# huangnengCSU/NanoSNP

Measured on AMD Instinct MI355X. Metric: candidate SNP sites/sec (pileup encode + model fwd), 30x windows, higher is better.
Workload: dtype f32; 1 GPU; BASELINE configs[1]: pileup encode + PileupModel fwd, 1M synthetic 30x windows (G2) resident in HBM, batch=4096; batch=4096, windows_resident_per_gpu=1048576, streams=32, precision=fp32, parallelism=site-sharded x1, rooted gather of calls, world_size_observed=1, gather=torch

## Files before the change

### nanosnp_amd/csrc/nsnp_api.hip

```cpp
#include "nsnp_common.hpp"

#include <new>

extern "C" int nsnp_version(void) { return 101; }

extern "C" const char* nsnp_strerror(int code)
{
    switch (code) {
    case NSNP_OK: return "ok";
    case NSNP_EINVAL: return "invalid argument";
    case NSNP_ENOMEM: return "out of memory";
    case NSNP_EHIP: return "HIP runtime error";
    case NSNP_ENOWEIGHTS: return "weights not loaded";
    case NSNP_EARCH: return "device is not gfx950";
    case NSNP_ESHAPE: return "unsupported model dimensions";
    case NSNP_ENOTSUP: return "optional component unavailable (RCCL not found)";
    case NSNP_ECOMM: return "RCCL call failed";
    default: return "unknown error";
    }
}

static hipError_t g_create_err = hipSuccess;

extern "C" int nsnp_last_hip_error(const nsnp_ctx* ctx, const char** text)
{
    const hipError_t e = ctx ? ctx->last_err : g_create_err;
    if (text) *text = hipGetErrorString(e);
    return (int)e;
}

extern "C" int nsnp_ctx_create(int device, nsnp_ctx** out)
{
    if (!out) return NSNP_EINVAL;
    *out = nullptr;
    nsnp_ctx* ctx = new (std::nothrow) nsnp_ctx();
    if (!ctx) return NSNP_ENOMEM;
    memset((void*)ctx, 0, sizeof(*ctx));
    ctx->device = device;
    ctx->last_err = hipSuccess;
    ctx->chunk_sites = 32768;
    ctx->hap_chunk = 16384;
    ctx->precision = 0;
    ctx->hap_precision = 0;
    ctx->cat_precision = 0;
    ctx->cat_conv_lds = 1;
    ctx->cat_conv_pix2 = 1;
    ctx->hap_b3x = 1;
    ctx->tok_fused = 0;
    ctx->proj1_tiles = 4;
    ctx->fused_l1 = 1;
    ctx->l0_rs = 2;
    ctx->l1_rs = 1;
    ctx->l1_stagger = 0;
    ctx->l1_weave = 1;
    ctx->head_rs = 1;
    ctx->rs_prio = 0;
    hipDeviceProp_t prop;
    hipError_t e = hipSetDevice(device);
    if (e == hipSuccess) e = hipGetDeviceProperties(&prop, device);
    if (e != hipSuccess) { g_create_err = e; delete ctx; return NSNP_EHIP; }
    if (strncmp(prop.gcnArchName, "gfx950", 6) != 0) { delete ctx; return NSNP_EARCH; }
    ctx->n_cu = prop.multiProcessorCount;
    *out = ctx;
    return NSNP_OK;
}

void nsnp_hap_free(nsnp_ctx* ctx);
int  nsnp_hap_reserve(nsnp_ctx* ctx);
void nsnp_cat_free(nsnp_ctx* ctx);
void nsnp_tok_free(nsnp_ctx* ctx);

constexpr size_t TIMER_MAX_PAIRS = 8192;

ScopedKernelTimer::ScopedKernelTimer(nsnp_ctx* c, int kernel, hipStream_t stream)
    : ctx(c), k(kernel), s(stream), stop_ev(nullptr), on(false)
{
    KernelTimer* t = c->timer;
    if (!t || !t->enabled || t->used[k] >= TIMER_MAX_PAIRS) return;
    if (t->used[k] == t->start[k].size()) {
        hipEvent_t a, b;
        if (hipEventCreate(&a) != hipSuccess) return;
        if (hipEventCreate(&b) != hipSuccess) { (void)hipEventDestroy(a); return; }
        t->start[k].push_back(a); t->stop[k].push_back(b);
    }
    const size_t i = t->used[k]++;
    (void)hipEventRecord(t->start[k][i], s);
    stop_ev = t->stop[k][i];
    on = true;
}
void ScopedKernelTimer::stop() { if (on) { (void)hipEventRecord(stop_ev, s); on = false; } }
ScopedKernelTimer::~ScopedKernelTimer() { stop(); }

extern "C" int nsnp_ctx_set_option(nsnp_ctx* ctx, const char* name, int64_t value)
{
    if (!ctx || !name) return NSNP_EINVAL;
    if (strcmp(name, "cat_precision") == 0) {
        if (value != 0 && value != 1 && value != 2) return NSNP_EINVAL;
        ctx->cat_precision = (int)value;
        return NSNP_OK;
    }
    if (strcmp(name, "tok_fused") == 0) {
        if (value != 0 && value != 1) return NSNP_EINVAL;
        ctx->tok_fused = (int)value;
        return NSNP_OK;
    }
    if (strcmp(name, "hap_b3x") == 0) {
        if (value != 0 && value != 1) return NSNP_EINVAL;
        ctx->hap_b3x = (int)value;
        return NSNP_OK;
    }
    if (strcmp(name, "cat_conv_pix2") == 0) {
        if (value != 0 && value != 1) return NSNP_EINVAL;
        ctx->cat_conv_pix2 = (int)value;
        return NSNP_OK;
    }
    if (strcmp(name, "cat_conv_lds") == 0) {
        if (value != 0 && value != 1) return NSNP_EINVAL;
        ctx->cat_conv_lds = (int)value;
        return NSNP_OK;
    }
    if (strcmp(name, "hap_precision") == 0) {
        if (value != 0 && value != 1 && value != 2) return NSNP_EINVAL;
        ctx->hap_precision = (int)value;
        return nsnp_hap_reserve(ctx);
    }
    if (strcmp(name, "hap_pass_sites") == 0) {
        if (value < 128 || value > 131072 || value % 128) return NSNP_EINVAL;
        const int64_t old = ctx->hap_chunk;
        ctx->hap_chunk = value;
        const int rc = nsnp_hap_reserve(ctx);
        if (rc) { ctx->hap_chunk = old; (void)nsnp_hap_reserve(ctx); }
        return rc;
    }
    if (strcmp(name, "pileup_precision") == 0) {
        if (value != 0 && value != 1 && value != 2) return NSNP_EINVAL;
        ctx->precision = (int)value;
        if (value == 2 && ctx->ws_h0 && ctx->ws_h0_floats < 192) return nsnp_ctx_reserve(ctx, ctx->chunk_sites);
        return NSNP_OK;
    }
    if (strcmp(name, "fused_l1") == 0) {
        if (value != 0 && value != 1) return NSNP_EINVAL;
        ctx->fused_l1 = (int)value;
        return NSNP_OK;
    }
    if (strcmp(name, "l0_register_stationary") == 0) {
        if (value != 0 && value != 1 && value != 2) return NSNP_EINVAL;
        ctx->l0_rs = (int)value;
        return NSNP_OK;
    }
    if (strcmp(name, "l1_register_stationary") == 0) {
        if (value != 0 && value != 1 && value != 2) return NSNP_EINVAL;
        ctx->l1_rs = (int)value;
        return NSNP_OK;
    }
    if (strcmp(name, "l0_input_weights_in_lds") == 0) {
        if (value != 0 && value != 1) return NSNP_EINVAL;
        ctx->l0_wx_lds = (int)value;
        return NSNP_OK;
    }
    if (strcmp(name, "static_priority") == 0) {
        if (value < 0 || value > 3) return NSNP_EINVAL;
        ctx->rs_prio = (int)value;
        return NSNP_OK;
    }
    if (strcmp(name, "head_split") == 0) {
        if (value != 0 && value != 1) return NSNP_EINVAL;
        ctx->head_rs = (int)value;
        return NSNP_OK;
    }
    if (strcmp(name, "l1_stagger") == 0) {
        if (value != 0 && value != 1) return NSNP_EINVAL;
        ctx->l1_stagger = (int)value;
        return NSNP_OK;
    }
    if (strcmp(name, "l1_weave") == 0) {
        if (value != 0 && value != 1) return NSNP_EINVAL;
        ctx->l1_weave = (int)value;
        return NSNP_OK;
    }
    if (strcmp(name, "l1_site_groups") == 0) {
        if (value != 0 && value != 1 && value != 2 && value != 4) return NSNP_EINVAL;
        ctx->l1_rs_groups = (int)value;
        return NSNP_OK;
    }
    if (strcmp(name, "l0_site_groups") == 0) {
        if (value != 0 && value != 1 && value != 2 && value != 4) return NSNP_EINVAL;
        ctx->l0_rs_groups = (int)value;
        return NSNP_OK;
    }
    if (strcmp(name, "fused_waves") == 0) {
        if (value != 0 && value != 4 && value != 8 && value != 12) return NSNP_EINVAL;
        ctx->fused_waves = (int)value;
        return NSNP_OK;
    }
    if (strcmp(name, "proj1_tiles") == 0) {
        if (value < 1 || value > 64) return NSNP_EINVAL;
        ctx->proj1_tiles = (int)value;
        return NSNP_OK;
    }
    if (strcmp(name, "recurrence_waves") == 0) {
        if (value != 0 && value != 1 && value != 2 && value != 4 && value != 8) return NSNP_EINVAL;
        ctx->force_wpb = (int)value;
        return NSNP_OK;
    }
    return NSNP_EINVAL;
}

extern "C" int nsnp_ctx_enable_timing(nsnp_ctx* ctx, int enable)
{
    if (!ctx) return NSNP_EINVAL;
    if (!ctx->timer) {
        ctx->timer = new (std::nothrow) KernelTimer();
        if (!ctx->timer) return NSNP_ENOMEM;
        for (int k = 0; k < NSNP_K_COUNT; ++k) ctx->timer->used[k] = 0;
    }
    ctx->timer->enabled = enable != 0;
    return NSNP_OK;
}

extern "C" int nsnp_ctx_read_timing(nsnp_ctx* ctx, int kernel, double* total_ms, int64_t* launches)
{
    if (!ctx || kernel < 0 || kernel >= NSNP_K_COUNT || !total_ms || !launches) return NSNP_EINVAL;
    *total_ms = 0.0; *launches = 0;
    KernelTimer* t = ctx->timer;
    if (!t) return NSNP_OK;
    for (size_t i = 0; i < t->used[kernel]; ++i) {
        NSNP_HIP(ctx, hipEventSynchronize(t->stop[kernel][i]));
        float ms = 0.f;
        NSNP_HIP(ctx, hipEventElapsedTime(&ms, t->start[kernel][i], t->stop[kernel][i]));
        *total_ms += ms; ++*launches;
    }
    t->used[kernel] = 0;
    return NSNP_OK;
}

static void free_ws(nsnp_ctx* ctx)
{
    if (ctx->ws_h0) (void)hipFree(ctx->ws_h0);
    if (ctx->ws_xp1) (void)hipFree(ctx->ws_xp1);
    if (ctx->ws_h1c) (void)hipFree(ctx->ws_h1c);
    ctx->ws_h0 = ctx->ws_xp1 = ctx->ws_h1c = nullptr;
    ctx->ws_h0_floats = 0;
}

extern "C" int nsnp_ctx_destroy(nsnp_ctx* ctx)
{
    if (!ctx) return NSNP_EINVAL;
    (void)hipSetDevice(ctx->device);
    (void)hipDeviceSynchronize();
    free_ws(ctx);
    if (ctx->pw.arena) (void)hipFree(ctx->pw.arena);
    if (ctx->pw16.arena) (void)hipFree(ctx->pw16.arena);
    if (ctx->pw16.l1f_bias) (void)hipFree(ctx->pw16.l1f_bias);
    if (ctx->pwb3.arena) (void)hipFree(ctx->pwb3.arena);
    if (ctx->sel_tmp) (void)hipFree(ctx->sel_tmp);
    if (ctx->fil_tmp) (void)hipFree(ctx->fil_tmp);
    if (ctx->rec_tmp) (void)hipFree(ctx->rec_tmp);
    if (ctx->lab_tmp) (void)hipFree(ctx->lab_tmp);
    if (ctx->evl_tmp) (void)hipFree(ctx->evl_tmp);
    if (ctx->pw.head6_w) (void)hipFree(ctx->pw.head6_w);
// ... 137 lines not shown
```

### nanosnp_amd/csrc/nsnp_common.hpp

```cpp
#pragma once

#include <hip/hip_runtime.h>
#include <stdint.h>
#include <stdlib.h>
#include <string.h>
#include <vector>

#include "nanosnp.h"

typedef float f32x4 __attribute__((ext_vector_type(4)));
typedef int   i32x4 __attribute__((ext_vector_type(4)));

#define NSNP_CDIV(a, b) (((a) + (b) - 1) / (b))

constexpr int PW = NSNP_PILEUP_WINDOW;
constexpr int PC = NSNP_PILEUP_CHANNELS;
constexpr int PH = 64;
constexpr int PG = 4 * PH;
constexpr int PCENTER = 16;
constexpr int PSTEPS1 = PCENTER + 1;


struct PileupWeightsDev {
    float* l0_whh[2];
    float* l0_wih[2];
    float* l0_wlast[2];
    void*  l0_wx[2];
    float* l1_wih[2];
    float* l1_bias[2];
    float* l1_bias_raw[2];
    float* l1_whh[2];
    float* proj_w;
    float* proj_b;
    float* dense_w;
    float* dense_b;
    float* head_w;
    float* head_b;
    float* arena;
    size_t arena_bytes;
    bool   loaded;
    float* head6_w;
    float* head6_b;
    bool   indel_loaded;
};

struct PileupWeightsF16 {
    void* l0_whh[2]; void* l0_wih_hi[2]; void* l0_wih_lo[2]; void* l1_wih[2]; void* l1_whh[2];
    void* l1f_hi[2]; void* l1f_lo[2]; float* l1f_bias;
    void* l0_wih_rs[2];
    void* l1_wih_rs[2]; void* l1_whh_rs[2];
    void* l0_whh_rs[2];
    void* proj_w; void* dense_w; void* head_w;
    void* arena; size_t arena_bytes; bool loaded;
};

struct PileupWeightsB3 {
    void* l0_whh[2]; void* l0_wih[2]; void* l1_wih[2]; void* l1_whh[2];
    void* proj_w; void* dense_w; void* head_w;
    float* proj_b; float* dense_b; float* head_b;
    void* arena; size_t arena_bytes; bool loaded;
};

struct HapWeightsDev;
struct CatWeightsDev;

enum { NSNP_K_L0 = 0, NSNP_K_PROJ1, NSNP_K_L1, NSNP_K_HEAD, NSNP_K_ENCODE, NSNP_K_HAPFEAT, NSNP_K_HAPLSTM, NSNP_K_CATCONV, NSNP_K_CAT,
       NSNP_K_COUNT };
struct KernelTimer {
    std::vector<hipEvent_t> start[NSNP_K_COUNT], stop[NSNP_K_COUNT];
    size_t used[NSNP_K_COUNT];
    bool enabled;
};

struct PostOut { uint8_t* gt_arg; uint8_t* zy_arg; float* gt_max; float* zy_max; };

struct nsnp_ctx {
    int device;
    int n_cu;
    hipError_t last_err;
    bool attr_set;
    bool attr_set_f16;
    bool attr_set_b3;
    int hap_b3x;
    int cat_conv_pix2;
    int cat_conv_lds;
    int cat_precision;
    int hap_precision;
    int precision;
    int fused_waves;
    int l0_rs;
    int l1_rs_groups;
    int l1_rs;
    int l0_rs_groups;
    int fused_l1;
    int proj1_tiles;
    int force_wpb;
    int l0_wx_lds;
    int rs_prio;
    int head_rs;
    int l1_stagger;
    int l1_weave;
    int64_t chunk_sites;
    float*  ws_h0;
    int     ws_h0_floats;
    float*  ws_xp1;
    float*  ws_h1c;
    PileupWeightsDev pw;
    PileupWeightsF16 pw16;
    PileupWeightsB3 pwb3;
    HapWeightsDev* hw;
    void*  hap_ws; size_t hap_ws_bytes; int64_t hap_ws_chunk;
    int64_t hap_chunk;
    CatWeightsDev* cw;
    void*  cat_ws; size_t cat_ws_bytes;
    int64_t* sel_tmp; size_t sel_tmp_bytes;
    int64_t* fil_tmp; size_t fil_tmp_bytes;
    void* rec_tmp; size_t rec_tmp_bytes;
    void* evl_tmp; size_t evl_tmp_bytes;
    void* lab_tmp; size_t lab_tmp_bytes;
    void* tok_ws; size_t tok_ws_bytes;
    void* ctg_ws; size_t ctg_ws_bytes;
    int tok_fused;
    bool af_cached; uint64_t af_bits, af_t; int af_k, af_mode; uint32_t af_table_words[128];
    bool af2_cached; uint64_t af2_bits, af2_t; int af2_k, af2_mode; uint32_t af2_table_words[128];
    KernelTimer* timer;
    void* comm; int comm_rank, comm_world;
    bool comm_borrowed;
};

struct ScopedKernelTimer {
    nsnp_ctx* ctx; int k; hipStream_t s; hipEvent_t stop_ev; bool on;
    ScopedKernelTimer(nsnp_ctx* c, int kernel, hipStream_t stream);
    void stop();
    ~ScopedKernelTimer();
};

#define NSNP_HIP(ctx, call)                                                        \
    do {                                                                           \
        hipError_t e_ = (call);                                                    \
        if (e_ != hipSuccess) { (ctx)->last_err = e_; return NSNP_EHIP; }          \
    } while (0)

typedef float (*nsnp_wfun)(const void* user, int row, int k);
void nsnp_pack_image(float* img, int n_tiles, int n_j4, nsnp_wfun f, const void* user);

int nsnp_ctx_need_xp1(nsnp_ctx* ctx);

int nsnp_pileup_forward_impl(nsnp_ctx* ctx, const int32_t* x, const int64_t* center_idx,
                             int64_t N, float* gt, float* zy, const PostOut* post, bool* post_written, hipStream_t s);
int nsnp_pileup_pack_weights(nsnp_ctx* ctx, const float* const* w);
int nsnp_pileup_pack_indel_heads(nsnp_ctx* ctx, const float* const* w);
int nsnp_pileup_eval_impl(nsnp_ctx* ctx, const int32_t* x, const int64_t* center_idx, const uint8_t* cls, int64_t N, float* site_loss,
                          uint8_t* pred, int64_t* counters, float* logits, hipStream_t s);
void nsnp_pileup_eval_heads_launch(nsnp_ctx* ctx, int64_t n, const uint8_t* cls, float* site_loss, uint8_t* pred, int64_t* counters,
                                   float* logits, hipStream_t s);
int nsnp_pileup_forward_f16x3(nsnp_ctx* ctx, const int32_t* x, const int64_t* center_idx,
                              int64_t N, float* gt, float* zy, hipStream_t s);
int nsnp_pileup_pack_weights_f16(nsnp_ctx* ctx, const float* const* w);
int nsnp_pileup_forward_bf16x3(nsnp_ctx* ctx, const int32_t* x, const int64_t* center_idx, int64_t N, float* gt, float* zy,
                               const PostOut* post, hipStream_t s);
int nsnp_pileup_pack_weights_bf16(nsnp_ctx* ctx, const float* const* w);
```

### nanosnp_amd/csrc/pileup_forward.hip

```cpp
#include "nsnp_common.hpp"
#include "nsnp_lstm_cell.hpp"
#include "nsnp_devclock.hpp"
#include "nsnp_bf16.hpp"
#include <type_traits>

namespace {

constexpr float LOG2E = 1.4426950408889634f;

__device__ __forceinline__ f32x4 mfma4(float a, float b, f32x4 c)
{
    return __builtin_amdgcn_mfma_f32_16x16x4f32(a, b, c, 0, 0, 0);
}
__device__ __forceinline__ float sigmoid_f(float x)
{
    return __builtin_amdgcn_rcpf(1.0f + __builtin_amdgcn_exp2f(-LOG2E * x));
}
__device__ __forceinline__ float tanh_f(float x)
{
    return __builtin_fmaf(-2.0f, __builtin_amdgcn_rcpf(1.0f + __builtin_amdgcn_exp2f((2.0f * LOG2E) * x)), 1.0f);
}

__device__ __forceinline__ float lstm_cell(float zi, float zf, float zg, float zo, float& c)
{
// ... 520 lines not shown
    for (int i = tid; i < 2 * 3 * RX_PLANE / 8; i += 256) reinterpret_cast<b8*>(&xx[0][0][0])[i] = b8{0, 0, 0, 0, 0, 0, 0, 0};
    if (tid < 8) xlvl[tid >> 2][tid & 3] = 0;
    __syncthreads();
    if (tid < 32) xx[tid >> 4][0][2 * 128 + (tid & 15) * 8 + 2] = (__bf16)1.0f;
    load_x(dir ? PW - 1 : 0);
    stage_x(0);
    if (PW > 1) load_x(dir ? PW - 2 : 1);
    __syncthreads();

    float c[4];
#pragma unroll
    for (int u = 0; u < 4; ++u) c[u] = 0.f;

    float* const h0wg = H0 + (base_site * PW * 2 + dir) * 64;
    const int frow = tid >> 4, fcid = tid & 15;
    unsigned foff = (unsigned)(frow * (PW * 128) + 4 * fcid) * 4u;
    const float* const fl = &hx[0][frow][16 * (fcid & 3) + 4 * (fcid >> 2)];
    const bool fon = frow < nrows;
    auto flush_h = [&](int buf, int t) {
        asm volatile("" : "+v"(foff));
        if (fon)
            *reinterpret_cast<f32x4*>(reinterpret_cast<char*>(h0wg + t * 128) + foff) =
                *reinterpret_cast<const f32x4*>(fl + buf * (16 * RS_XROW));
    };

    for (int s = 0; s < PW; ++s) {
        const int t = dir ? PW - 1 - s : s;
        const int cur = s & 1;
        if (s > 0) flush_h(cur ^ 1, dir ? t + 1 : t - 1);
        const __bf16* xr = &xx[cur][0][q * 128 + n * 8];
        const b8 xb0 = *reinterpret_cast<const b8*>(xr);
        const i32x4 lv = *reinterpret_cast<const i32x4*>(xlvl[cur]);
        const int lvl = __builtin_amdgcn_readfirstlane(max(max(lv[0], lv[1]), max(lv[2], lv[3])));
        f32x4 hn;
        auto step = [&](auto lvl_tag) __attribute__((always_inline)) {
            constexpr int LVL = decltype(lvl_tag)::value;
            const float* hr = &hx[cur ^ 1][n][4 * q];
            f32x4 hb0, hb1;
            if (s > 0) { hb0 = *reinterpret_cast<const f32x4*>(hr); hb1 = *reinterpret_cast<const f32x4*>(hr + 16); }
            f32x4 acc[4];
#pragma unroll
            for (int u = 0; u < 4; ++u) acc[u] = f32x4{0.f, 0.f, 0.f, 0.f};
#pragma unroll
            for (int p = LVL; p >= 0; --p) {
                const b8 b = p ? *reinterpret_cast<const b8*>(xr + p * RX_PLANE) : xb0;
#pragma unroll
                for (int wp = 2; wp >= 0; --wp)
#pragma unroll
                    for (int u = 0; u < 4; ++u) acc[u] = __builtin_amdgcn_mfma_f32_16x16x32_bf16(Wx[u][wp], b, acc[u], 0, 0, 0);
            }
            if (s > 0) {
#define RS_KBLOCK(J, HB)                                                                               \
                _Pragma("unroll") for (int e = 0; e < 4; ++e)                                          \
                    _Pragma("unroll") for (int u = 0; u < 4; ++u) acc[u] = mfma4(Whh[u][J][e], HB[e], acc[u]);
                __builtin_amdgcn_sched_barrier(0);
                RS_KBLOCK(0, hb0)
                __builtin_amdgcn_sched_barrier(0);
                hb0 = *reinterpret_cast<const f32x4*>(hr + 32);
                RS_KBLOCK(1, hb1)
                __builtin_amdgcn_sched_barrier(0);
                hb1 = *reinterpret_cast<const f32x4*>(hr + 48);
                RS_KBLOCK(2, hb0)
                __builtin_amdgcn_sched_barrier(0);
                RS_KBLOCK(3, hb1)
#undef RS_KBLOCK
            }
#pragma unroll
            for (int u = 0; u < 4; ++u) hn[u] = lstm_cell(acc[u][0], acc[u][1], acc[u][2], acc[u][3], c[u]);
        };
        if (__builtin_expect(lvl == 0, 1)) step(std::integral_constant<int, 0>{});
        else if (lvl == 1)                 step(std::integral_constant<int, 1>{});
        else                               step(std::integral_constant<int, 2>{});
        *reinterpret_cast<f32x4*>(&hx[cur][n][16 * wave + 4 * q]) = hn;
        if (s + 1 < PW) {
            stage_x(cur ^ 1);
            if (s + 2 < PW) load_x(dir ? t - 2 : t + 2);
        }
        lds_barrier();
    }
    flush_h((PW - 1) & 1, dir ? 0 : PW - 1);
    NSNP_DEVCLK_STOP(0)
}

constexpr int rs32_l1_lds_bytes(int nsg) { return (2 * 16 * nsg * RS_H0ROW + 2 * 16 * nsg * RS_XROW) * 4; }

template <int NSG, bool STAGGER>
__global__ __launch_bounds__(512, 2) void k_pileup_l1_rs32(
    const float* __restrict__ H0, int64_t N,
    const float* __restrict__ wih0, const float* __restrict__ wih1,
    const float* __restrict__ whh0, const float* __restrict__ whh1,
    const float* __restrict__ bias0, const float* __restrict__ bias1,
    float* __restrict__ H1c)
{
    extern __shared__ f32x4 lds[];
    constexpr int NS = 16 * NSG;
    float* const h0s = reinterpret_cast<float*>(lds);
    float* const h1x = h0s + 2 * NS * RS_H0ROW;
    const int dir = blockIdx.y;
    const int tid = threadIdx.x, lane = tid & 63, wave = tid >> 6;
    const int n = lane & 15, q = lane >> 4;
    const int64_t base_site = (int64_t)blockIdx.x * NS;

    f32x4 Wih[2][8], Whh[2][4], bias[2];
    {
        const f32x4* __restrict__ gih = reinterpret_cast<const f32x4*>(dir ? wih1 : wih0);
        const f32x4* __restrict__ ghh = reinterpret_cast<const f32x4*>(dir ? whh1 : whh0);
        const f32x4* __restrict__ gb = reinterpret_cast<const f32x4*>(dir ? bias1 : bias0);
#pragma unroll
        for (int u = 0; u < 2; ++u) {
#pragma unroll
            for (int j = 0; j < 8; ++j) Wih[u][j] = gih[((2 * wave + u) * 8 + j) * 64 + lane];
#pragma unroll
            for (int j = 0; j < 4; ++j) Whh[u][j] = ghh[((2 * wave + u) * 4 + j) * 64 + lane];
            bias[u] = gb[(2 * wave + u) * 64 + lane];
        }
    }

    const int cid = tid & 31;
    const int slot = (cid & 16) + 4 * (cid & 3) + ((cid >> 2) & 3);
    f32x4 sreg[NSG];
    auto load_h0 = [&](int t) {
#pragma unroll
        for (int k = 0; k < NSG; ++k) {
            const int64_t site = base_site + (tid >> 5) + 16 * k;
            const int64_t sc = site < N ? site : N - 1;
            sreg[k] = *reinterpret_cast<const f32x4*>(H0 + (sc * PW + t) * 128 + 4 * cid);
        }
    };
    auto store_h0 = [&](int buf) {
#pragma unroll
        for (int k = 0; k < NSG; ++k)
            *reinterpret_cast<f32x4*>(h0s + ((size_t)buf * NS + (tid >> 5) + 16 * k) * RS_H0ROW + 4 * slot) = sreg[k];
    };
    auto tpos = [&](int u) { return dir ? PW - 1 - u : u; };
    load_h0(tpos(0)); store_h0(0);
    load_h0(tpos(1)); store_h0(1);
    __syncthreads();
    load_h0(tpos(2));

    f32x4 acc[NSG][2];
    auto input_part = [&](int sg, int buf, f32x4& a0, f32x4& a1) {
        const float* r0 = h0s + ((size_t)buf * NS + 16 * sg + n) * RS_H0ROW + 4 * q;
        a0 = bias[0]; a1 = bias[1];
#pragma unroll
        for (int j = 0; j < 8; ++j) {
            const f32x4 b4 = *reinterpret_cast<const f32x4*>(r0 + 64 * (j >> 2) + 16 * (j & 3));
#pragma unroll
            for (int e = 0; e < 4; ++e) {
                a0 = mfma4(Wih[0][j][e], b4[e], a0);
                a1 = mfma4(Wih[1][j][e], b4[e], a1);
            }
        }
    };
    const bool late = STAGGER && wave >= 4;
#pragma unroll
    for (int sg = 0; sg < NSG; ++sg) input_part(sg, 0, acc[sg][0], acc[sg][1]);
    lds_barrier();

    float c[NSG][2];
#pragma unroll
    for (int sg = 0; sg < NSG; ++sg) c[sg][0] = c[sg][1] = 0.f;

    for (int s = 0; s < PSTEPS1; ++s) {
        const int cur = s & 1;
        const float* hrb = h1x + (size_t)(cur ^ 1) * NS * RS_XROW;
        float* hwb = h1x + (size_t)cur * NS * RS_XROW;
// ... 85 lines not shown
            const int64_t site = base_site + (tid >> 5) + 8 * k;
            const int64_t sc = site < N ? site : N - 1;
            sreg[k] = *reinterpret_cast<const f32x4*>(H0 + (sc * PW + t) * 128 + 4 * cid);
        }
    };
    auto store_h0 = [&](int buf) {
#pragma unroll
        for (int k = 0; k < 2 * NSG; ++k)
            *reinterpret_cast<f32x4*>(h0s + ((size_t)buf * NS + (tid >> 5) + 8 * k) * RS_H0ROW + 4 * slot) = sreg[k];
    };
    load_h0(dir ? PW - 1 : 0);
    store_h0(0);
    if (PSTEPS1 > 1) load_h0(dir ? PW - 2 : 1);
    __syncthreads();

    float c[NSG][4];
#pragma unroll
    for (int sg = 0; sg < NSG; ++sg)
#pragma unroll
        for (int u = 0; u < 4; ++u) c[sg][u] = 0.f;

    for (int s = 0; s < PSTEPS1; ++s) {
        const int t = dir ? PW - 1 - s : s;
        const int cur = s & 1;
        const float* h0b = h0s + (size_t)cur * NS * RS_H0ROW;
        const float* hrb = h1x + (size_t)(cur ^ 1) * NS * RS_XROW;
        float* hwb = h1x + (size_t)cur * NS * RS_XROW;
#pragma unroll
        for (int sg = 0; sg < NSG; ++sg) {
            const float* r0 = h0b + (size_t)(16 * sg + n) * RS_H0ROW + 4 * q;
            f32x4 acc[4];
#pragma unroll
            for (int u = 0; u < 4; ++u) acc[u] = lbias[(4 * wave + u) * 4 + q];
#pragma unroll
            for (int j = 0; j < 8; ++j) {
                if (sg == 0 && j == 2 && s + 1 < PSTEPS1) {
                    __builtin_amdgcn_sched_barrier(0);
                    store_h0(cur ^ 1);
                    __builtin_amdgcn_sched_barrier(0);
                }
                if (sg == 0 && j == 5 && s + 2 < PSTEPS1) {
                    __builtin_amdgcn_sched_barrier(0);
                    load_h0(dir ? t - 2 : t + 2);
                    __builtin_amdgcn_sched_barrier(0);
                }
                const f32x4 b4 = *reinterpret_cast<const f32x4*>(r0 + 64 * (j >> 2) + 16 * (j & 3));
#pragma unroll
                for (int e = 0; e < 4; ++e)
#pragma unroll
                    for (int u = 0; u < 4; ++u) acc[u] = mfma4(Wih[u][j][e], b4[e], acc[u]);
            }
            if (s > 0) {
                const float* r1 = hrb + (size_t)(16 * sg + n) * RS_XROW + 4 * q;
#pragma unroll
                for (int j = 0; j < 4; ++j) {
                    const f32x4 b4 = *reinterpret_cast<const f32x4*>(r1 + 16 * j);
#pragma unroll
                    for (int e = 0; e < 4; ++e)
#pragma unroll
                        for (int u = 0; u < 4; ++u) acc[u] = mfma4(Whh[u][j][e], b4[e], acc[u]);
                }
            }
            f32x4 hn;
#pragma unroll
            for (int u = 0; u < 4; ++u) {
                hn[u] = lstm_cell(acc[u][0], acc[u][1], acc[u][2], acc[u][3], c[sg][u]);
            }
            *reinterpret_cast<f32x4*>(hwb + (size_t)(16 * sg + n) * RS_XROW + 16 * wave + 4 * q) = hn;
        }
        lds_barrier();
    }
    const float* hfin = h1x + (size_t)((PSTEPS1 - 1) & 1) * NS * RS_XROW;
#pragma unroll
    for (int sg = 0; sg < NSG; ++sg) {
        const int64_t site = base_site + 16 * sg + n;
        if (site < N)
            *reinterpret_cast<f32x4*>(H1c + site * 128 + dir * 64 + q * 16 + 4 * wave) =
                *reinterpret_cast<const f32x4*>(hfin + (size_t)(16 * sg + n) * RS_XROW + 16 * wave + 4 * q);
    }
    NSNP_DEVCLK_STOP(1)
}

constexpr int rs4w_l1_lds_bytes() { return rs4_l1_lds_bytes(1) + 4 * 4 * 2 * 64 * 16; }

template <int... I, class F>
__device__ __forceinline__ void static_for_seq(std::integer_sequence<int, I...>, F&& f) { (f(std::integral_constant<int, I>{}), ...); }
template <int N, class F>
__device__ __forceinline__ void static_for(F&& f) { static_for_seq(std::make_integer_sequence<int, N>{}, f); }

template <int CELL_PER_GAP, int CELL_FIRST_GAP>
__global__ __launch_bounds__(256, 2) void k_pileup_l1_rs4w(
    const float* __restrict__ H0, int64_t N,
    const float* __restrict__ wih0, const float* __restrict__ wih1,
    const float* __restrict__ whh0, const float* __restrict__ whh1,
    const float* __restrict__ bias0, const float* __restrict__ bias1,
    float* __restrict__ H1c)
{
    extern __shared__ f32x4 lds[];
    float* const h0s = reinterpret_cast<float*>(lds);
    float* const h1x = h0s + 2 * 16 * RS_H0ROW;
    f32x4* const lbias = reinterpret_cast<f32x4*>(h1x + 2 * 16 * RS_XROW);
    f32x4* const lwhh = lbias + 64;
    const int dir = blockIdx.y;
    const int tid = threadIdx.x, lane = tid & 63, wave = tid >> 6;
    const int n = lane & 15, q = lane >> 4;
    NSNP_DEVCLK_START
    const int64_t base_site = (int64_t)blockIdx.x * 16;

    f32x4 Wih[4][8], Whh[4][2];
    f32x4* const lw = lwhh + wave * (4 * 2 * 64) + lane;
    {
        const f32x4* __restrict__ gih = reinterpret_cast<const f32x4*>(dir ? wih1 : wih0);
        const f32x4* __restrict__ ghh = reinterpret_cast<const f32x4*>(dir ? whh1 : whh0);
#pragma unroll
        for (int u = 0; u < 4; ++u) {
#pragma unroll
            for (int j = 0; j < 8; ++j) Wih[u][j] = gih[((4 * wave + u) * 8 + j) * 64 + lane];
#pragma unroll
            for (int j = 0; j < 2; ++j) Whh[u][j] = ghh[((4 * wave + u) * 4 + j) * 64 + lane];
#pragma unroll
            for (int j = 0; j < 2; ++j) lw[(2 * u + j) * 64] = ghh[((4 * wave + u) * 4 + 2 + j) * 64 + lane];
        }
        if (tid < 64) lbias[tid] = reinterpret_cast<const f32x4*>(dir ? bias1 : bias0)[(tid >> 2) * 64 + 16 * (tid & 3)];
    }

    const int cid = tid & 31;
    const int slot = (cid & 16) + 4 * (cid & 3) + ((cid >> 2) & 3);
    f32x4 sreg[2];
    const float* const h0wg = H0 + base_site * (PW * 128);
    unsigned hoff[2];
#pragma unroll
    for (int k = 0; k < 2; ++k) {
        const int64_t site = base_site + (tid >> 5) + 8 * k;
        const int64_t sc = site < N ? site : N - 1;
        hoff[k] = (unsigned)((int)(sc - base_site) * (PW * 128) + 4 * cid) * 4u;
    }
    auto tpos = [&](int u) { return dir ? PW - 1 - u : u; };
    auto load_h0 = [&](int t) {
#pragma unroll
        for (int k = 0; k < 2; ++k) {
            asm volatile("" : "+v"(hoff[k]));
            sreg[k] = *reinterpret_cast<const f32x4*>(reinterpret_cast<const char*>(h0wg + t * 128) + hoff[k]);
        }
    };
    auto store_h0 = [&](int buf) {
#pragma unroll
        for (int k = 0; k < 2; ++k)
            *reinterpret_cast<f32x4*>(h0s + ((size_t)buf * 16 + (tid >> 5) + 8 * k) * RS_H0ROW + 4 * slot) = sreg[k];
    };
    static_assert(PSTEPS1 >= 3, "the pipeline stages three steps in its prologue");
    load_h0(tpos(0)); store_h0(0);
    load_h0(tpos(1)); store_h0(1);
    __syncthreads();
    load_h0(tpos(2));

    float c[4];
#pragma unroll
    for (int u = 0; u < 4; ++u) c[u] = 0.f;

    auto project_reads = [&](int buf, f32x4 (&p)[4], f32x4& b0) __attribute__((always_inline)) {
        b0 = *reinterpret_cast<const f32x4*>(h0s + ((size_t)buf * 16 + n) * RS_H0ROW + 4 * q);
#pragma unroll
        for (int u = 0; u < 4; ++u) p[u] = lbias[(4 * wave + u) * 4 + q];
    };
    auto project = [&](int buf, f32x4 (&p)[4], const f32x4& b0, auto cell_tag, f32x4 (&a)[4], float* hout, int tnext)
                       __attribute__((always_inline)) {
        constexpr bool CELL = decltype(cell_tag)::value;
        constexpr int NGAPS = (nsnp_cell::CELL_SLICES + CELL_PER_GAP - 1) / CELL_PER_GAP, CELL_END = CELL_FIRST_GAP + NGAPS;
        static_assert(CELL_END + 8 <= 128, "the cell, the h1 row and the h0 staging end inside the burst");
        const float* r0 = h0s + ((size_t)buf * 16 + n) * RS_H0ROW + 4 * q;
        f32x4 b4[2];
// ... 460 lines not shown
    if (pw.arena && pw.arena_bytes != total * sizeof(float)) { (void)hipFree(pw.arena); pw.arena = nullptr; }
    if (!pw.arena) {
        NSNP_HIP(ctx, hipMalloc((void**)&pw.arena, total * sizeof(float)));
        pw.arena_bytes = total * sizeof(float);
    }
    NSNP_HIP(ctx, hipMemcpy(pw.arena, host.data(), total * sizeof(float), hipMemcpyHostToDevice));
    auto dev = [&](const float* hp) { return pw.arena + (hp - host.data()); };
    for (int d = 0; d < 2; ++d) {
        pw.l0_whh[d] = dev(h_l0_whh[d]); pw.l0_wih[d] = dev(h_l0_wih[d]); pw.l0_wlast[d] = dev(h_l0_wlast[d]);
        pw.l0_wx[d] = dev(h_l0_wx[d]);
        pw.l1_wih[d] = dev(h_l1_wih[d]); pw.l1_bias[d] = dev(h_l1_b[d]); pw.l1_bias_raw[d] = dev(h_l1_braw[d]); pw.l1_whh[d] = dev(h_l1_whh[d]);
    }
    pw.proj_w = dev(h_proj); pw.proj_b = dev(h_pb); pw.dense_w = dev(h_dense); pw.dense_b = dev(h_db);
    pw.head_w = dev(h_head); pw.head_b = dev(h_hb);
    pw.loaded = true;
    pw.indel_loaded = false;
    return NSNP_OK;
}

int nsnp_pileup_pack_indel_heads(nsnp_ctx* ctx, const float* const* w)
{
    PileupWeightsDev& pw = ctx->pw;
    constexpr size_t n_w = 6 * 16 * 256, n_b = 6 * 256;
    std::vector<float> img(n_w), bias(n_b), old_w(2 * 16 * 256), old_b(2 * 256);
    NSNP_HIP(ctx, hipDeviceSynchronize());
    NSNP_HIP(ctx, hipMemcpy(old_w.data(), pw.head_w, old_w.size() * sizeof(float), hipMemcpyDeviceToHost));
    NSNP_HIP(ctx, hipMemcpy(old_b.data(), pw.head_b, old_b.size() * sizeof(float), hipMemcpyDeviceToHost));
    struct IndelRef { const float* w1; const float* w2; } ir{w[0], w[2]};
    nsnp_pack_image(img.data(), 6, 16, [](const void* u, int row, int k) -> float {
        const IndelRef* m = (const IndelRef*)u;
        if (row >= 24 && row < 57) return m->w1[(row - 24) * 256 + acc_col(k)];
        if (row >= 57 && row < 90) return m->w2[(row - 57) * 256 + acc_col(k)];
        return 0.f;
    }, &ir);
    for (int tile = 0; tile < 2; ++tile) for (int j4 = 0; j4 < 16; ++j4) for (int lane = 0; lane < 64; ++lane)
        if (16 * tile + (lane & 15) < 24)
            for (int e = 0; e < 4; ++e) img[((tile * 16 + j4) * 64 + lane) * 4 + e] = old_w[((tile * 16 + j4) * 64 + lane) * 4 + e];
    for (int tile = 0; tile < 6; ++tile) for (int lane = 0; lane < 64; ++lane) for (int g = 0; g < 4; ++g) {
        const int row = 16 * tile + 4 * (lane >> 4) + g;
        bias[(tile * 64 + lane) * 4 + g] = row < 24 ? old_b[(tile * 64 + lane) * 4 + g] : (row < 57 ? w[1][row - 24] : (row < 90 ? w[3][row - 57] : 0.f));
    }
    if (!pw.head6_w) NSNP_HIP(ctx, hipMalloc((void**)&pw.head6_w, n_w * sizeof(float)));
    if (!pw.head6_b) NSNP_HIP(ctx, hipMalloc((void**)&pw.head6_b, n_b * sizeof(float)));
    NSNP_HIP(ctx, hipMemcpy(pw.head6_w, img.data(), n_w * sizeof(float), hipMemcpyHostToDevice));
    NSNP_HIP(ctx, hipMemcpy(pw.head6_b, bias.data(), n_b * sizeof(float), hipMemcpyHostToDevice));
    pw.indel_loaded = true;
    return NSNP_OK;
}

static int set_lds_attr_once(nsnp_ctx* ctx)
{
    if (ctx->attr_set) return NSNP_OK;
    NSNP_HIP(ctx, hipFuncSetAttribute((const void*)k_pileup_l0<8>, hipFuncAttributeMaxDynamicSharedMemorySize, L0_LDS_BYTES));
    NSNP_HIP(ctx, hipFuncSetAttribute((const void*)k_pileup_l0<4>, hipFuncAttributeMaxDynamicSharedMemorySize, L0_LDS_BYTES));
    NSNP_HIP(ctx, hipFuncSetAttribute((const void*)k_pileup_l0<2>, hipFuncAttributeMaxDynamicSharedMemorySize, L0_LDS_BYTES));
    NSNP_HIP(ctx, hipFuncSetAttribute((const void*)k_pileup_l0<1>, hipFuncAttributeMaxDynamicSharedMemorySize, L0_LDS_BYTES));
    NSNP_HIP(ctx, hipFuncSetAttribute((const void*)k_pileup_proj1, hipFuncAttributeMaxDynamicSharedMemorySize, P1_LDS_BYTES));
    NSNP_HIP(ctx, hipFuncSetAttribute((const void*)k_pileup_l1<8>, hipFuncAttributeMaxDynamicSharedMemorySize, L1_LDS_BYTES));
    NSNP_HIP(ctx, hipFuncSetAttribute((const void*)k_pileup_l1<4>, hipFuncAttributeMaxDynamicSharedMemorySize, L1_LDS_BYTES));
    NSNP_HIP(ctx, hipFuncSetAttribute((const void*)k_pileup_l1<2>, hipFuncAttributeMaxDynamicSharedMemorySize, L1_LDS_BYTES));
    NSNP_HIP(ctx, hipFuncSetAttribute((const void*)k_pileup_l1<1>, hipFuncAttributeMaxDynamicSharedMemorySize, L1_LDS_BYTES));
    NSNP_HIP(ctx, hipFuncSetAttribute((const void*)k_pileup_l1_rs4<1>, hipFuncAttributeMaxDynamicSharedMemorySize, rs4_l1_lds_bytes(1)));
    NSNP_HIP(ctx, hipFuncSetAttribute((const void*)k_pileup_l1_rs4<2>, hipFuncAttributeMaxDynamicSharedMemorySize, rs4_l1_lds_bytes(2)));
    NSNP_HIP(ctx, hipFuncSetAttribute((const void*)k_pileup_l1_rs4w<RS4W_PER_GAP, RS4W_FIRST_GAP>, hipFuncAttributeMaxDynamicSharedMemorySize, rs4w_l1_lds_bytes()));
    NSNP_HIP(ctx, hipFuncSetAttribute((const void*)k_pileup_l1_rs32<4, true>, hipFuncAttributeMaxDynamicSharedMemorySize, rs32_l1_lds_bytes(4)));
    NSNP_HIP(ctx, hipFuncSetAttribute((const void*)k_pileup_l1_rs32<2, true>, hipFuncAttributeMaxDynamicSharedMemorySize, rs32_l1_lds_bytes(2)));
    NSNP_HIP(ctx, hipFuncSetAttribute((const void*)k_pileup_l1_rs32<4, false>, hipFuncAttributeMaxDynamicSharedMemorySize, rs32_l1_lds_bytes(4)));
    NSNP_HIP(ctx, hipFuncSetAttribute((const void*)k_pileup_l1_rs32<2, false>, hipFuncAttributeMaxDynamicSharedMemorySize, rs32_l1_lds_bytes(2)));
    ctx->attr_set = true;
    return NSNP_OK;
}

static int launch_layers(nsnp_ctx* ctx, const int32_t* xc, const int64_t* cc, int64_t n, hipStream_t s)
{
    const PileupWeightsDev& pw = ctx->pw;
    {
        const int64_t waves_total = NSNP_CDIV(n, 16) * 2;
        int wpb = 8;
        while (wpb > 1 && waves_total / wpb < (int64_t)ctx->n_cu / 2) wpb >>= 1;
        if (ctx->force_wpb) wpb = ctx->force_wpb;
        const dim3 g_rec((unsigned)NSNP_CDIV(n, 16 * wpb), 2);
        if (ctx->l0_rs == 2) {
            ScopedKernelTimer tm(ctx, NSNP_K_L0, s);
            hipLaunchKernelGGL(k_pileup_l0_rsx, dim3((unsigned)NSNP_CDIV(n, 16), 2), dim3(256), 0, s, xc, cc, n,
                               pw.l0_whh[0], pw.l0_whh[1], (const __bf16*)pw.l0_wx[0], (const __bf16*)pw.l0_wx[1], ctx->ws_h0);
        } else if (ctx->l0_rs) {
            ScopedKernelTimer tm(ctx, NSNP_K_L0, s);
            int nsg = 1;
            if (ctx->l0_rs_groups) nsg = ctx->l0_rs_groups;
#define LAUNCH_RS(G) hipLaunchKernelGGL(k_pileup_l0_rs32<G>, dim3((unsigned)NSNP_CDIV(n, 16 * G), 2), dim3(256), 0, s, xc, cc, n, \
                           pw.l0_whh[0], pw.l0_whh[1], pw.l0_wih[0], pw.l0_wih[1], pw.l0_wlast[0], pw.l0_wlast[1], ctx->ws_h0)
            if (ctx->l0_wx_lds && nsg == 1)
                hipLaunchKernelGGL((k_pileup_l0_rs32<1, true>), dim3((unsigned)NSNP_CDIV(n, 16), 2), dim3(256), 0, s, xc, cc, n,
                                   pw.l0_whh[0], pw.l0_whh[1], pw.l0_wih[0], pw.l0_wih[1], pw.l0_wlast[0], pw.l0_wlast[1], ctx->ws_h0);
            else
            if (nsg == 4) LAUNCH_RS(4); else if (nsg == 2) LAUNCH_RS(2); else LAUNCH_RS(1);
#undef LAUNCH_RS
        } else
        { ScopedKernelTimer tm(ctx, NSNP_K_L0, s);
#define LAUNCH_L0(W) hipLaunchKernelGGL(k_pileup_l0<W>, g_rec, dim3(64 * W), L0_LDS_BYTES, s, xc, cc, n, \
                           pw.l0_whh[0], pw.l0_whh[1], pw.l0_wih[0], pw.l0_wih[1], pw.l0_wlast[0], pw.l0_wlast[1], ctx->ws_h0)
        if (wpb == 8) LAUNCH_L0(8); else if (wpb == 4) LAUNCH_L0(4); else if (wpb == 2) LAUNCH_L0(2); else LAUNCH_L0(1);
#undef LAUNCH_L0
        }
        if (ctx->l1_rs == 1) {
            ScopedKernelTimer tm(ctx, NSNP_K_L1, s);
            int g1 = 1;
            if (ctx->l1_rs_groups == 1 || ctx->l1_rs_groups == 2) g1 = ctx->l1_rs_groups;
#define LAUNCH_R4(G) hipLaunchKernelGGL(k_pileup_l1_rs4<G>, dim3((unsigned)NSNP_CDIV(n, 16 * G), 2), dim3(256), rs4_l1_lds_bytes(G), s, \
                           ctx->ws_h0, n, pw.l1_wih[0], pw.l1_wih[1], pw.l1_whh[0], pw.l1_whh[1], pw.l1_bias[0], pw.l1_bias[1], ctx->ws_h1c)
            if (g1 == 2) LAUNCH_R4(2);
            else if (ctx->l1_weave)
                hipLaunchKernelGGL((k_pileup_l1_rs4w<RS4W_PER_GAP, RS4W_FIRST_GAP>), dim3((unsigned)NSNP_CDIV(n, 16), 2), dim3(256),
                                   rs4w_l1_lds_bytes(), s, ctx->ws_h0, n, pw.l1_wih[0], pw.l1_wih[1], pw.l1_whh[0], pw.l1_whh[1],
                                   pw.l1_bias[0], pw.l1_bias[1], ctx->ws_h1c);
            else LAUNCH_R4(1);
#undef LAUNCH_R4
        } else if (ctx->l1_rs == 2) {
            ScopedKernelTimer tm(ctx, NSNP_K_L1, s);
            int g1 = NSNP_CDIV(n, 64) * 2 >= (int64_t)ctx->n_cu ? 4 : 2;
            if (ctx->l1_rs_groups) g1 = ctx->l1_rs_groups;
#define LAUNCH_R1(G) hipLaunchKernelGGL((k_pileup_l1_rs32<G, ST>), dim3((unsigned)NSNP_CDIV(n, 16 * G), 2), dim3(512), rs32_l1_lds_bytes(G), s, \
                           ctx->ws_h0, n, pw.l1_wih[0], pw.l1_wih[1], pw.l1_whh[0], pw.l1_whh[1], pw.l1_bias[0], pw.l1_bias[1], ctx->ws_h1c)
            if (ctx->l1_stagger) { constexpr bool ST = true; if (g1 == 4) LAUNCH_R1(4); else LAUNCH_R1(2); }
            else { constexpr bool ST = false; if (g1 == 4) LAUNCH_R1(4); else LAUNCH_R1(2); }
#undef LAUNCH_R1
        } else {
        { const int rx = nsnp_ctx_need_xp1(ctx); if (rx) return rx; }
        const int64_t n_rt = NSNP_CDIV(n * PSTEPS1, 16);
        int64_t gp = NSNP_CDIV(n_rt, 16 * (int64_t)ctx->proj1_tiles);
        if (gp > ctx->n_cu) gp = ctx->n_cu;
        if (gp < 1) gp = 1;
        { ScopedKernelTimer tm(ctx, NSNP_K_PROJ1, s);
        hipLaunchKernelGGL(k_pileup_proj1, dim3((unsigned)gp, 2), dim3(1024), P1_LDS_BYTES, s, ctx->ws_h0, n,
                           pw.l1_wih[0], pw.l1_wih[1], pw.l1_bias[0], pw.l1_bias[1], ctx->ws_xp1); }
        { ScopedKernelTimer tm(ctx, NSNP_K_L1, s);
#define LAUNCH_L1(W) hipLaunchKernelGGL(k_pileup_l1<W>, g_rec, dim3(64 * W), L1_LDS_BYTES, s, ctx->ws_xp1, n, \
                           pw.l1_whh[0], pw.l1_whh[1], ctx->ws_h1c)
        if (wpb == 8) LAUNCH_L1(8); else if (wpb == 4) LAUNCH_L1(4); else if (wpb == 2) LAUNCH_L1(2); else LAUNCH_L1(1);
#undef LAUNCH_L1
        }
        }
    }
    return NSNP_OK;
}

int nsnp_pileup_forward_impl(nsnp_ctx* ctx, const int32_t* x, const int64_t* center_idx,
                             int64_t N, float* gt, float* zy, const PostOut* post, bool* post_written, hipStream_t s)
{
    if (!ctx->pw.loaded) return NSNP_ENOWEIGHTS;
    if (N == 0) return NSNP_OK;
    int rc = set_lds_attr_once(ctx);
    if (rc) return rc;
    if (!ctx->ws_h0) { rc = nsnp_ctx_reserve(ctx, ctx->chunk_sites); if (rc) return rc; }
    const PileupWeightsDev& pw = ctx->pw;
    for (int64_t base = 0; base < N; base += ctx->chunk_sites) {
        const int64_t n = (N - base < ctx->chunk_sites) ? N - base : ctx->chunk_sites;
        const int32_t* xc = center_idx ? x : x + base * (PW * PC);
        const int64_t* cc = center_idx ? center_idx + base : nullptr;
        rc = launch_layers(ctx, xc, cc, n, s);
        if (rc) return rc;
        ScopedKernelTimer tm_head(ctx, NSNP_K_HEAD, s);
        if (ctx->head_rs) {
            int64_t gh = NSNP_CDIV(n, 16);
            if (gh > 2 * (int64_t)ctx->n_cu) gh = 2 * (int64_t)ctx->n_cu;
            const PostOut po = post ? *post : PostOut{nullptr, nullptr, nullptr, nullptr};
// ... 49 lines not shown
```

Baseline: 20.75 million sites/s.

## Add software-pipelined layer-0 LSTM kernel weaving next-step input MFMAs into cell math

Adds a new layer-0 recurrent kernel that interleaves the next timestep's input-projection MFMAs (bf16) into the elementwise LSTM cell computation, paced by a compile-time schedule so matrix and vector/transcendental work overlap. It also prefetches inputs three steps ahead, flushes hidden states mid-step, and splits large input values across extra bf16 planes only when needed. The new kernel is enabled by default through a new l0_weave knob. It trades heavier register pressure (launch bounds of 3 blocks) and rigid sched_barrier scheduling for hiding MFMA latency behind cell math.

```diff
diff --git a/nanosnp_amd/csrc/nsnp_api.hip b/nanosnp_amd/csrc/nsnp_api.hip
--- a/nanosnp_amd/csrc/nsnp_api.hip
+++ b/nanosnp_amd/csrc/nsnp_api.hip
@@ -50,6 +50,7 @@
     ctx->proj1_tiles = 4;
     ctx->fused_l1 = 1;
     ctx->l0_rs = 2;
+    ctx->l0_weave = 1;
     ctx->l1_rs = 1;
     ctx->l1_stagger = 0;
     ctx->l1_weave = 1;
@@ -176,6 +177,11 @@
     if (strcmp(name, "l1_weave") == 0) {
         if (value != 0 && value != 1) return NSNP_EINVAL;
         ctx->l1_weave = (int)value;
+        return NSNP_OK;
+    }
+    if (strcmp(name, "l0_weave") == 0) {
+        if (value != 0 && value != 1) return NSNP_EINVAL;
+        ctx->l0_weave = (int)value;
         return NSNP_OK;
     }
     if (strcmp(name, "l1_site_groups") == 0) {
diff --git a/nanosnp_amd/csrc/nsnp_common.hpp b/nanosnp_amd/csrc/nsnp_common.hpp
--- a/nanosnp_amd/csrc/nsnp_common.hpp
+++ b/nanosnp_amd/csrc/nsnp_common.hpp
@@ -99,6 +99,7 @@
     int rs_prio;
     int head_rs;
     int l1_stagger;
+    int l0_weave;
     int l1_weave;
     int64_t chunk_sites;
     float*  ws_h0;
diff --git a/nanosnp_amd/csrc/pileup_forward.hip b/nanosnp_amd/csrc/pileup_forward.hip
--- a/nanosnp_amd/csrc/pileup_forward.hip
+++ b/nanosnp_amd/csrc/pileup_forward.hip
@@ -626,6 +626,249 @@
     NSNP_DEVCLK_STOP(0)
 }
 
+template <int... I, class F>
+__device__ __forceinline__ void static_for_seq(std::integer_sequence<int, I...>, F&& f) { (f(std::integral_constant<int, I>{}), ...); }
+template <int N, class F>
+__device__ __forceinline__ void static_for(F&& f) { static_for_seq(std::make_integer_sequence<int, N>{}, f); }
+
+constexpr bool rsxw_slice_is_trans(int i)
+{
+    const int st = i >> 2;
+    return st == 0 || st == 1 || st == 2 || st == 4 || st == 7 || st == 11 || st == 14 || st == 17;
+}
+constexpr int rsxw_late_slice(int k) { return k < 8 ? 4 * (5 + (k & 1)) + (k >> 1) : 20 + k; }
+constexpr int rsxw_mfmas_upto(int gap_t, int gap_v, int first, int nm, int last)
+{
+    int m = 0, run = 0;
+    for (int k = first; k <= last; ++k) {
+        const int quota = rsxw_slice_is_trans(rsxw_late_slice(k)) ? gap_t : gap_v;
+        if (quota == 0) continue;
+        if (m < nm && (m == 0 || run >= quota)) { ++m; run = 0; }
+        ++run;
+    }
+    return m;
+}
+
+template <int GAP_T, int GAP_V, int GAP_FIRST, bool LATE_W0>
+__global__ __launch_bounds__(256, 3) void k_pileup_l0_rsxw(
+    const int32_t* __restrict__ x, const int64_t* __restrict__ center_idx, int64_t N,
+    const float* __restrict__ whh0, const float* __restrict__ whh1,
+    const __bf16* __restrict__ wx0, const __bf16* __restrict__ wx1,
+    float* __restrict__ H0)
+{
+    static_assert(GAP_T == 0 || GAP_V == 0, "one class of cell instruction paces the burst");
+    static_assert(PW >= 3, "the pipeline stages three steps in its prologue");
+    __shared__ __attribute__((aligned(16))) float hx[3][16][RS_XROW];
+    __shared__ __attribute__((aligned(16))) __bf16 xx[2][3][RX_PLANE];
+    __shared__ __attribute__((aligned(16))) int xlvl[2][4];
+    const int dir = blockIdx.y;
+    const int tid = threadIdx.x, lane = tid & 63, wave = __builtin_amdgcn_readfirstlane(tid >> 6);
+    const int n = lane & 15, q = lane >> 4;
+    NSNP_DEVCLK_START
+    const int64_t base_site = (int64_t)blockIdx.x * 16;
+    const int nrows = (int)min((int64_t)16, N - base_site);
+
+    f32x4 Whh[4][4];
+    b8 Wx[4][3];
+    {
+        const f32x4* __restrict__ ghh = reinterpret_cast<const f32x4*>(dir ? whh1 : whh0);
+        const b8* __restrict__ gx = reinterpret_cast<const b8*>(dir ? wx1 : wx0);
+#pragma unroll
+        for (int u = 0; u < 4; ++u) {
+#pragma unroll
+            for (int j = 0; j < 4; ++j) Whh[u][j] = ghh[((4 * wave + u) * 4 + j) * 64 + lane];
+#pragma unroll
+            for (int p = 0; p < 3; ++p) Wx[u][p] = gx[((4 * wave + u) * 3 + p) * 64 + lane];
+        }
+    }
+    const bool xon = tid < 9 * 16;
+    const int xrow = min(wave < 2 ? lane >> 2 : n, nrows - 1);
+    const int piece = wave < 2 ? 4 * wave + (lane & 3) : 8;
+    const int xdst = wave < 2 ? 128 * wave + 2 * lane : 256 + 8 * n;
+    const int frow = tid >> 4, fcid = tid & 15;
+    float* const fl = &hx[0][frow][16 * (fcid & 3) + 4 * (fcid >> 2)];
+    int64_t* const xofs = reinterpret_cast<int64_t*>(fl + 2 * 16 * RS_XROW);
+    if (xon) *xofs = (center_idx ? (center_idx[base_site + xrow] - PCENTER) * PC : (base_site + xrow) * (PW * PC)) + 2 * piece;
+    int2 xi = int2{0, 0};
+    auto tpos = [&](int u) { return dir ? PW - 1 - u : u; };
+    auto load_x = [&](int t) {
+        if (!xon) return;
+        xi = *reinterpret_cast<const int2*>(x + *xofs + t * PC);
+    };
+    auto stage_x_split = [&](b2* d, int* lv) {
+        __bf16 a0, a1, a2, c0, c1, c2;
+        split3((float)xi.x, a0, a1, a2); split3((float)xi.y, c0, c1, c2);
+        d[0] = b2{a0, c0}; d[RX_PLANE / 2] = b2{a1, c1}; d[RX_PLANE] = b2{a2, c2};
+        const bool nz1 = (float)a1 != 0.f || (float)c1 != 0.f, nz2 = (float)a2 != 0.f || (float)c2 != 0.f;
+        const int lvl = __ballot(nz2) != 0ull ? 2 : (__ballot(nz1) != 0ull ? 1 : 0);
+        if (lane == 0) *lv = lvl;
+    };
+    auto stage_x = [&](int buf) {
+        if (!xon) return;
+        b2* const d = reinterpret_cast<b2*>(&xx[buf][0][xdst]);
+        const bool big = (unsigned)xi.x + 256u > 512u || (unsigned)xi.y + 256u > 512u;
+        if (__builtin_expect(__ballot(big) == 0ull, 1)) {
+            d[0] = __builtin_convertvector(f32x2{(float)xi.x, (float)xi.y}, b2);
+            d[RX_PLANE / 2] = b2{0, 0};
+            d[RX_PLANE] = b2{0, 0};
+            if (lane == 0) xlvl[buf][wave] = 0;
+        } else {
+            stage_x_split(d, &xlvl[buf][wave]);
+        }
+    };
+    for (int i = tid; i < 2 * 3 * RX_PLANE / 8; i += 256) reinterpret_cast<b8*>(&xx[0][0][0])[i] = b8{0, 0, 0, 0, 0, 0, 0, 0};
+    if (tid < 8) xlvl[tid >> 2][tid & 3] = 0;
+    __syncthreads();
+    if (tid < 32) xx[tid >> 4][0][2 * 128 + (tid & 15) * 8 + 2] = (__bf16)1.0f;
+    load_x(tpos(0)); stage_x(0);
+    load_x(tpos(1)); stage_x(1);
+    load_x(tpos(2));
+    __syncthreads();
+
+    float c[4];
+#pragma unroll
+    for (int u = 0; u < 4; ++u) c[u] = 0.f;
+
+    float* const h0wg = H0 + (base_site * PW * 2 + dir) * 64;
+    unsigned foff = (unsigned)(frow * (PW * 128) + 4 * fcid) * 4u;
+    const bool fon = frow < nrows;
+    auto flush_h = [&](int buf, int t) {
+        asm volatile("" : "+v"(foff));
+        if (fon)
+            *reinterpret_cast<f32x4*>(reinterpret_cast<char*>(h0wg + t * 128) + foff) =
+                *reinterpret_cast<const f32x4*>(fl + buf * (16 * RS_XROW));
+    };
+
+    constexpr int NM = LATE_W0 ? 8 : 12;
+    auto read_x = [&](int buf, b8& xb0, int& lvl) __attribute__((always_inline)) {
+        xb0 = *reinterpret_cast<const b8*>(&xx[buf][0][q * 128 + n * 8]);
+        const i32x4 lv = *reinterpret_cast<const i32x4*>(xlvl[buf]);
+        lvl = __builtin_amdgcn_readfirstlane(max(max(lv[0], lv[1]), max(lv[2], lv[3])));
+    };
+    auto project_block = [&](int buf, const b8& xb0, f32x4 (&acc)[4], auto lvl_tag) __attribute__((always_inline)) {
+        constexpr int LVL = decltype(lvl_tag)::value;
+        const __bf16* xr = &xx[buf][0][q * 128 + n * 8];
+#pragma unroll
+        for (int u = 0; u < 4; ++u) acc[u] = f32x4{0.f, 0.f, 0.f, 0.f};
+#pragma unroll
+        for (int p = LVL; p >= 0; --p) {
+            const b8 b = p ? *reinterpret_cast<const b8*>(xr + p * RX_PLANE) : xb0;
+#pragma unroll
+            for (int wp = 2; wp >= (LATE_W0 && p == 0 ? 1 : 0); --wp)
+#pragma unroll
+                for (int u = 0; u < 4; ++u) {
+                    acc[u] = __builtin_amdgcn_mfma_f32_16x16x32_bf16(Wx[u][wp], b, acc[u], 0, 0, 0);
+                    __builtin_amdgcn_sched_barrier(0);
+                }
+        }
+    };
+    auto project_any = [&](int buf, const b8& xb0, int lvl, f32x4 (&acc)[4]) __attribute__((always_inline)) {
+        if (__builtin_expect(lvl == 0, 1)) project_block(buf, xb0, acc, std::integral_constant<int, 0>{});
+        else if (lvl == 1)                 project_block(buf, xb0, acc, std::integral_constant<int, 1>{});
+        else                               project_block(buf, xb0, acc, std::integral_constant<int, 2>{});
+    };
+
+    f32x4 acc[4];
+    b8 xb;
+    {
+        int lvl0;
+        read_x(0, xb, lvl0);
+        project_any(0, xb, lvl0, acc);
+    }
+    lds_barrier();
+
+    auto step = [&](int s, auto first_tag, auto last_tag) __attribute__((always_inline)) {
+        constexpr bool FIRST = decltype(first_tag)::value, LAST = decltype(last_tag)::value;
+        const int t = tpos(s);
+        const int cur = s & 1;
+        const float* hr = &hx[cur ^ 1][n][4 * q];
+        f32x4 hb0, hb1;
+        if constexpr (!FIRST) { hb0 = *reinterpret_cast<const f32x4*>(hr); hb1 = *reinterpret_cast<const f32x4*>(hr + 16); }
+        if constexpr (LATE_W0) {
+            __builtin_amdgcn_sched_barrier(0);
+#pragma unroll
+            for (int u = 0; u < 4; ++u) acc[u] = __builtin_amdgcn_mfma_f32_16x16x32_bf16(Wx[u][0], xb, acc[u], 0, 0, 0);
+            __builtin_amdgcn_sched_barrier(0);
+        }
+        int lvln = 0;
+        if constexpr (FIRST) read_x(cur ^ 1, xb, lvln);
+        else {
+#define RSXW_KBLOCK(J, HB)                                                                             \
+            _Pragma("unroll") for (int e = 0; e < 4; ++e)                                              \
+                _Pragma("unroll") for (int u = 0; u < 4; ++u) acc[u] = mfma4(Whh[u][J][e], HB[e], acc[u]);
+            __builtin_amdgcn_sched_barrier(0);
+            RSXW_KBLOCK(0, hb0)
+            __builtin_amdgcn_sched_barrier(0);
+            hb0 = *reinterpret_cast<const f32x4*>(hr + 32);
+            RSXW_KBLOCK(1, hb1)
+            __builtin_amdgcn_sched_barrier(0);
+            hb1 = *reinterpret_cast<const f32x4*>(hr + 48);
+            if constexpr (!LAST) read_x(cur ^ 1, xb, lvln);
+            RSXW_KBLOCK(2, hb0)
+            __builtin_amdgcn_sched_barrier(0);
+            flush_h(cur ^ 1, dir ? t + 1 : t - 1);
+            RSXW_KBLOCK(3, hb1)
+#undef RSXW_KBLOCK
+        }
+        __builtin_amdgcn_sched_barrier(0);
+        nsnp_cell::CellSlices w;
+        f32x4 hn;
+        static_for<20>([&](auto ic) __attribute__((always_inline)) {
+            constexpr int k = decltype(ic)::value, u = k / 5, st = k % 5 == 0 ? 3 : k % 5 == 4 ? 4 : k % 5 - 1;
+            nsnp_cell::lstm_cell_slice<4 * st + u>(w, acc, c, hn);
+        });
+        __builtin_amdgcn_sched_barrier(0);
+        auto burst = [&](auto from_tag, auto to_tag) __attribute__((always_inline)) {
+            constexpr int FROM = decltype(from_tag)::value, TO = decltype(to_tag)::value;
+            if constexpr (!LAST)
+                static_for<TO - FROM>([&](auto mc) __attribute__((always_inline)) {
+                    constexpr int m = FROM + decltype(mc)::value, u = m & 3, wp = 2 - (m >> 2);
+                    if constexpr (m < 4) acc[u] = f32x4{0.f, 0.f, 0.f, 0.f};
+                    acc[u] = __builtin_amdgcn_mfma_f32_16x16x32_bf16(Wx[u][wp], xb, acc[u], 0, 0, 0);
+                    __builtin_amdgcn_sched_barrier(0);
+                });
+        };
+        static_for<60>([&](auto kc) __attribute__((always_inline)) {
+            constexpr int k = decltype(kc)::value;
+            constexpr int before = rsxw_mfmas_upto(GAP_T, GAP_V, GAP_FIRST, NM, k - 1), upto = rsxw_mfmas_upto(GAP_T, GAP_V, GAP_FIRST, NM, k);
+            burst(std::integral_constant<int, before>{}, std::integral_constant<int, upto>{});
+            nsnp_cell::lstm_cell_slice<rsxw_late_slice(k)>(w, acc, c, hn);
+            __builtin_amdgcn_sched_barrier(0);
+        });
+        *reinterpret_cast<f32x4*>(&hx[cur][n][16 * wave + 4 * q]) = hn;
+        __builtin_amdgcn_sched_barrier(0);
+        burst(std::integral_constant<int, rsxw_mfmas_upto(GAP_T, GAP_V, GAP_FIRST, NM, 59)>{}, std::integral_constant<int, NM>{});
+        if constexpr (!LAST) {
+            if (__builtin_expect(lvln != 0, 0)) {
+                if (lvln == 1) project_block(cur ^ 1, xb, acc, std::integral_constant<int, 1>{});
+                else           project_block(cur ^ 1, xb, acc, std::integral_constant<int, 2>{});
+            }
+        }
+        if constexpr (!LAST) {
+            stage_x(cur);
+            load_x(tpos(s + 3 < PW ? s + 3 : PW - 1));
+        }
+        lds_barrier();
+    };
+    step(0, std::true_type{}, std::false_type{});
+    for (int s = 1; s < PW - 1; ++s) step(s, std::false_type{}, std::false_type{});
+    step(PW - 1, std::false_type{}, std::true_type{});
+    flush_h((PW - 1) & 1, dir ? 0 : PW - 1);
+    NSNP_DEVCLK_STOP(0)
+}
+#ifndef RSXW_GAP_T
+#define RSXW_GAP_T 1
+#endif
+#ifndef RSXW_GAP_V
+#define RSXW_GAP_V 0
+#endif
+#ifndef RSXW_GAP_FIRST
+#define RSXW_GAP_FIRST 24
+#endif
+#ifndef RSXW_LATE_W0
+#define RSXW_LATE_W0 1
+#endif
+
 constexpr int rs32_l1_lds_bytes(int nsg) { return (2 * 16 * nsg * RS_H0ROW + 2 * 16 * nsg * RS_XROW) * 4; }
 
 template <int NSG, bool STAGGER>
@@ -877,11 +1120,6 @@
 }
 
 constexpr int rs4w_l1_lds_bytes() { return rs4_l1_lds_bytes(1) + 4 * 4 * 2 * 64 * 16; }
-
-template <int... I, class F>
-__device__ __forceinline__ void static_for_seq(std::integer_sequence<int, I...>, F&& f) { (f(std::integral_constant<int, I>{}), ...); }
-template <int N, class F>
-__device__ __forceinline__ void static_for(F&& f) { static_for_seq(std::make_integer_sequence<int, N>{}, f); }
 
 template <int CELL_PER_GAP, int CELL_FIRST_GAP>
 __global__ __launch_bounds__(256, 2) void k_pileup_l1_rs4w(
@@ -1508,6 +1746,10 @@
         const dim3 g_rec((unsigned)NSNP_CDIV(n, 16 * wpb), 2);
         if (ctx->l0_rs == 2) {
             ScopedKernelTimer tm(ctx, NSNP_K_L0, s);
+            if (ctx->l0_weave)
+                hipLaunchKernelGGL((k_pileup_l0_rsxw<RSXW_GAP_T, RSXW_GAP_V, RSXW_GAP_FIRST, RSXW_LATE_W0 != 0>), dim3((unsigned)NSNP_CDIV(n, 16), 2), dim3(256), 0, s,
+                                   xc, cc, n, pw.l0_whh[0], pw.l0_whh[1], (const __bf16*)pw.l0_wx[0], (const __bf16*)pw.l0_wx[1], ctx->ws_h0);
+            else
             hipLaunchKernelGGL(k_pileup_l0_rsx, dim3((unsigned)NSNP_CDIV(n, 16), 2), dim3(256), 0, s, xc, cc, n,
                                pw.l0_whh[0], pw.l0_whh[1], (const __bf16*)pw.l0_wx[0], (const __bf16*)pw.l0_wx[1], ctx->ws_h0);
         } else if (ctx->l0_rs) {
```

Result: faster. 21.06 million sites/s, median of 6 (+1.5%).
